# TINY-KE/DSP-SLAM-RGBD

Hardware: AMD Instinct MI355X
Metric: object-reconstructions/sec (2048 pts, 10 GN iters) (higher is better)
Workload: dtype fp16-mfma: 3xFP16 split (hi/lo fp16, fp32 accumulate) for every value that reaches an output + one-product fp16 classification of ray samples

## Files before the change

dsp-slam-rgbd_amd/csrc/dsr_api.hip:

```cpp
#include <hip/hip_runtime.h>
#include <rccl/rccl.h>
#include <dlfcn.h>

#include <algorithm>
#include <chrono>
#include <climits>
#include <cmath>
#include <cstdio>
#include <cstring>
#include <functional>
#include <map>
#include <mutex>
#include <string>
#include <thread>
#include <vector>

#include "../../include/dsr.h"
#include "dsr_kernels.hpp"
#include "dsr_mc.hpp"

#ifndef DSR_DEFAULT_FWD_VARIANT
#define DSR_DEFAULT_FWD_VARIANT 12
#endif

// ... 28 lines not shown

static bool test_hooks() {
  const char* e = getenv("DSR_TEST_HOOKS");
  return e && atoi(e) != 0;
}
static const char* hook_env(const char* k) { return test_hooks() ? getenv(k) : nullptr; }

#ifndef DSR_DEFAULT_SPLIT_RING
#define DSR_DEFAULT_SPLIT_RING 2
#endif
static int split_ring() {
  const char* e = hook_env("DSR_SPLIT_RING");
  const int r = e ? atoi(e) : DSR_DEFAULT_SPLIT_RING;
  return (r >= 2 && r <= 4) ? r : 0;
}
using FwdKernel = void (*)(DevDecoder, const Tile*, const int*, const ObjDesc*, const float4*, const float*,
                           const float*, float*, unsigned*, ErtArgs, MaskArgs);
template <int MSK>
static FwdKernel fwd16_kernel() {
  switch (split_ring()) {
    case 2: return k_mlp_fwd16<true, MSK | 1024>;
    case 3: return k_mlp_fwd16<true, MSK | 2048>;
    case 4: return k_mlp_fwd16<true, MSK | 3072>;
  }
  return k_mlp_fwd16<true, MSK>;
}
static FwdKernel fwd_kernel(int v) {
  switch (v & 15) {
    case 1: return k_mlp_fwd<1>;
    case 2: return k_mlp_fwd<2>;
    case 3: return k_mlp_fwd<3>;
    case 6: return k_mlp_fwd<6>;
    case 7: return k_mlp_fwd<7>;
    case 8: return k_mlp_fwd16<false, 0>;
    case 12: return fwd16_kernel<0>();
    default: return k_mlp_fwd<0>;
  }
}
using JacKernel = void (*)(DevDecoder, const Tile*, const int*, const ObjDesc*, const ObjState*, const float*,
                           const float4*, const float*, const float*, const float*, GNParams, float*,
                           const float4*, float*, float*, MaskArgs, float*);
static int jac_variant();
static JacKernel jac_kernel() {
  const int v = jac_variant();
  switch (v) {
    case 8: return k_mlp_jac16<false, 0>;
    case 12:
      switch (split_ring()) {
        case 2: return k_mlp_jac16<true, 2>;
        case 3: return k_mlp_jac16<true, 3>;
        case 4: return k_mlp_jac16<true, 4>;
      }
      return k_mlp_jac16<true, 0>;
  }
  return k_mlp_jac;
}
static bool is_variant(const DevDecoder& D) { return D.xyz_all || D.use_tanh || D.ln_mask; }
static FwdKernel fwd_kernel_for(const DevDecoder& D, int v) {
  return is_variant(D) ? k_mlp_fwd16<true, 1024 | 8192> : fwd_kernel(v);
}
static JacKernel jac_kernel_for(const DevDecoder& D) {
  return is_variant(D) ? k_mlp_jac16<true, 2, true> : jac_kernel();
}
using LiteKernel = void (*)(DevDecoder, const Tile*, const int*, const ObjDesc*, const float4*, const float*,
// ... 116 lines not shown
  uint64_t *rbits = nullptr, *abits = nullptr;
  MaskArgs ma{nullptr, nullptr, nullptr, nullptr};
  int* kslot = nullptr;
  bool lite = true;
  int loop_iters = 0;
  bool spare_run = false;
  ErtArgs lite_cfg{};
  bool hooks = false;
  int* diag = nullptr;
  std::vector<int> passes;
  std::vector<hipEvent_t> ev;
  bool ran = false;
  int runs = 0;
  bool timed = false;
  bool prescan = false;
  int ran_fwd = 0, ran_jac = 0, ran_lite = 0, ran_ring = 0;
#ifdef DSR_EXP_PROV
  int *prov_alive = nullptr, *prov_set = nullptr, *prov_xcc = nullptr, *prov_j = nullptr;
  unsigned* prov_t = nullptr;
  unsigned* prov_h = nullptr;
  unsigned* prov_ri = nullptr;
  float* prov_nrm = nullptr;
  float* prov_nrm2 = nullptr;
  float* prov_y = nullptr;
  int prov_R = 0, prov_C = 0;
#endif
  hipGraphExec_t graph = nullptr;
  long graph_key = -1;
  int captures = 0, replays = 0;
  bool capacity = false;
  bool cap_graph = false;
// ... 1060 lines not shown
  return 0;
}

static int batch_enqueue(dsr_batch* b, bool timing = true);
static int batch_finish(dsr_batch* b);

static int jac_variant() {
  const char* e = hook_env("DSR_JAC_VARIANT");
  return e ? atoi(e) : 12;
}

static bool graph_enabled() {
  const char* ge = getenv("DSR_GRAPH");
  return ge && atoi(ge) != 0;
}
static long graph_key() { return ((long)fwd_variant() * 100000 + jac_variant()) * 10 + split_ring(); }

static int batch_capture(dsr_batch* b) {
  dsr_ctx* ctx = b->ctx;
  if (b->graph) {
    hipGraphExecDestroy(b->graph);
    b->graph = nullptr;
  }
  hipGraph_t g = nullptr;
  DSR_CHECK(ctx, hipStreamBeginCapture(ctx->stream, hipStreamCaptureModeThreadLocal));
  const int rc = batch_enqueue(b, false);
  const hipError_t ec = hipStreamEndCapture(ctx->stream, &g);
  if (rc) {
    if (g) hipGraphDestroy(g);
    return rc;
  }
// ... 113 lines not shown
  const GNParams P = b->P;
  const int grid = ctx->n_cu;
  const int cb = (n + 63) / 64;
  const int fv = fwd_variant();
  const FwdKernel fwdk = fwd_kernel_for(D, fv);
  const JacKernel jack = jac_kernel_for(D);
  const LiteKernel litek = lite_kernel();
  {
    const int fl = fv & 15;
    const bool known = fl == 1 || fl == 2 || fl == 3 || fl == 6 || fl == 7 || fl == 8 || fl == 12;
    const int jv = jac_variant();
    b->ran_fwd = is_variant(D) ? 12 : (known ? fv : (fv & ~15));
    b->ran_jac = is_variant(D) ? 12 : ((jv == 8 || jv == 12) ? jv : 0);
    b->ran_lite = b->lite ? lite_variant_dispatched() : 0;
    b->ran_ring = is_variant(D) ? 2 : split_ring();
  }
  const int np = (int)b->passes.size() - 1;
  const size_t epi = ev_per_iter(b);
  const int G = (int)b->groups.size();
  DSR_CHECK(ctx, hipEventRecord(b->fork_ev, s0));
  for (int g = 1; g < G; ++g) DSR_CHECK(ctx, hipStreamWaitEvent(ctx->gstream[g], b->fork_ev, 0));
  for (int it = it0; it < it1; ++it) {
    for (int g = 0; g < G; ++g) {
      const dsr_batch::Group& gr = b->groups[g];
      hipStream_t s = ctx->gstream[g];
      const int ng = gr.n, o0 = gr.o0;
      const ObjDesc* desc = b->desc + o0;
      ObjState* st = b->st + o0;
      float* zbuf = b->zbuf + (size_t)o0 * CODE;
      float* b0 = b->bias0f + (size_t)o0 * HID;
// ... 161 lines not shown
  st->lite_eligible = b->dec->info.lite_eligible;
  st->audit = (b->lite && b->lite_cfg.audit) ? 1 : 0;
  st->audit_shell = b->lite_cfg.shell;
  st->audit_log2 = b->lite_cfg.audit_log2;
  st->lite_margin0 = b->P.lite_margin0;
  st->lite_floor = b->P.lite_floor;
  st->lite_safety = b->P.lite_safety;
  st->graph_captures = b->captures;
  st->graph_replays = b->replays;
  st->n_groups = (int)b->groups.size();
  st->graph_mode = b->cap_graph ? 2 : (graph_enabled() ? 1 : 0);
  st->fwd_variant = b->ran_fwd;
  st->jac_variant = b->ran_jac;
  st->lite_variant = b->ran_lite;
  st->split_ring = b->ran_ring;
  st->prescan = b->prescan ? 1 : 0;
  {
    int nb = 0;
    DSR_CHECK(b->ctx, hipMemcpy(&nb, b->diag + STD_BROKEN, sizeof(int), hipMemcpyDeviceToHost));
    st->lite_broken_blocks = nb;
  }
  st->keep_masks = (b->lite && b->ma.msk && b->ran_fwd == 12) ? 1 : 0;
  st->surface_in_exact = (st->keep_masks && b->ma.pts && b->ran_jac == 12) ? 1 : 0;
  if (b->lite) {
    st->lite_min_margin = 1e30;
    for (const ObjState& o : hs) {
      st->lite_max_err = std::max(st->lite_max_err, (double)o.lite_err);
      if (o.iters_done > 0) st->lite_min_margin = std::min(st->lite_min_margin, (double)o.lite_margin);
      st->lite_audit_violations += o.lite_viol_total;
      st->lite_redo_objects += o.lite_redo ? 1 : 0;
// ... 834 lines not shown
```

dsp-slam-rgbd_amd/csrc/dsr_kernels.hpp:

```cpp
#pragma once
#include "dsr_dev.hpp"
#include "dsr_mlp.hpp"
#include "dsr_mlp16.hpp"
#include "dsr_mlp_lite.hpp"
#include "../../include/dsr.h"

extern "C" __device__ __attribute__((const)) unsigned long long __ockl_wfred_max_u64(unsigned long long);

namespace dsr {

template <int N>
__device__ __forceinline__ void lu_small(float (&a)[N][N], int (&piv)[N]) {
#pragma unroll
  for (int k = 0; k < N; ++k) {
    int p = k;
    float best = fabsf(a[k][k]);
#pragma unroll
    for (int r = k + 1; r < N; ++r)
      if (fabsf(a[r][k]) > best) { best = fabsf(a[r][k]); p = r; }
    piv[k] = p;
#pragma unroll
    for (int r = k + 1; r < N; ++r) {
      const bool sw = (p == r);
#pragma unroll
// ... 1314 lines not shown
  }
}

struct Jac16Shared {
  _Float16 Hh[TILE * PH];
  _Float16 Hl[TILE * PH];
  float xyz[TILE * 4];
  float red[NWAVE * TILE];
  float red2[NWAVE * TILE];
  float y[TILE];
  float r[TILE];
  float gin[TILE * GIN_PITCH];
  float wmax[NWAVE];
};

#if defined(DSR_EXP_NOLS)
constexpr int BWD_LS = 0;
#elif defined(DSR_EXP_BLS1)
constexpr int BWD_LS = 1;
#else
constexpr int BWD_LS = 2;
#endif

#ifdef DSR_EXP_STAMP
#define JSTAMP(cat)                                                         \
  {                                                                         \
    __builtin_amdgcn_sched_barrier(0);                                      \
    const unsigned long long t_ = __builtin_amdgcn_s_memtime();            \
    jstamp[cat] += t_ - jstamp_last;                                        \
    jstamp_last = t_;                                                       \
    __builtin_amdgcn_sched_barrier(0);                                      \
  }
#else
#define JSTAMP(cat)
#endif
template <bool PRIO, int NB, bool VAR = false>
__global__ __launch_bounds__(512) void k_mlp_jac16(DevDecoder D, const Tile* __restrict__ tiles,
                                                   const int* __restrict__ n_tiles,
                                                   const ObjDesc* __restrict__ desc,
                                                   const ObjState* __restrict__ st,
                                                   const float* __restrict__ pts_all,
                                                   const float4* __restrict__ kpts,
                                                   const float* __restrict__ kres,
                                                   const float* __restrict__ bias0f,
                                                   const float* __restrict__ bias4f, GNParams P,
                                                   float* __restrict__ slots,
                                                   const float4* __restrict__ raw_pts,
                                                   float* __restrict__ raw_out,
                                                   float* __restrict__ res_out, MaskArgs MA,
                                                   float* __restrict__ lnws) {
  __shared__ Jac16Shared sm;
  const int w = __builtin_amdgcn_readfirstlane(threadIdx.x >> 6);
  float* const lnw = lnws ? lnws + (size_t)blockIdx.x * LN_WS_WG : nullptr;
  const int nt = *n_tiles;
#ifdef DSR_EXP_STAMP
  unsigned long long jstamp[8] = {0, 0, 0, 0, 0, 0, 0, 0};
  unsigned long long jstamp_last = __builtin_amdgcn_s_memtime();
  int jtiles = 0;
#endif
  for (int ti = blockIdx.x; ti < nt; ti += gridDim.x) {
    const Tile tl = tiles[ti];
    const ObjDesc d = desc[tl.obj];
#ifdef DSR_EXP_STAMP
    ++jtiles;
#endif
    float zpre = 0.f;
    {
      const int tid = opaque(threadIdx.x);
      if (tid < TILE) {
        float x = 0.f, y = 0.f, z = 0.f, aux = 0.f, rr = 0.f;
        zpre = bias0f[tl.obj * HID];
        if (tid < tl.count) {
          if (tl.term == 0) {
            const float* p = pts_all + (size_t)(d.pts_off + tl.start + tid) * 3;
            const float3 xo = xform(st[tl.obj].T, p[0], p[1], p[2]);
            x = xo.x; y = xo.y; z = xo.z;
          } else if (tl.term == 1) {
            const float4 v = kpts[d.cand_off + tl.start + tid];
            x = v.x; y = v.y; z = v.z; aux = v.w;
            rr = kres[d.cand_off + tl.start + tid];
          } else {
            const float4 v = raw_pts[tl.start + tid];
// ... 2 lines not shown
        }
        *reinterpret_cast<float4*>(sm.xyz + tid * 4) = make_float4(x, y, z, aux);
        sm.r[tid] = rr;
      }
    }
    __syncthreads();
    uint64_t mk[8];
    float v[4][4][4];
    floatx4 acc[4][4];
    int sa;
    Scales2 fs;
    bool fast = false;
    if (MA.kslot != nullptr && tl.term == 1) {
      const int tid = opaque(threadIdx.x);
      int bad = 0;
      if (tid < tl.count) bad = MA.kslot[d.cand_off + tl.start + tid] < 0;
      fast = !__syncthreads_or(bad);
    } else if (MA.pts != nullptr && tl.term == 0) {
      fast = true;
    }
    auto mslot = [&](int p) {
      return tl.term == 1 ? d.cand_off + MA.kslot[d.cand_off + tl.start + p] : MA.surf_base + d.pts_off + tl.start + p;
    };
    if (fast) {
      const int lane = opaque(threadIdx.x & 63), g = lane >> 4, c = lane & 15;
#pragma unroll
      for (int l = 0; l < 8; ++l) mk[l] = 0;
#pragma unroll
      for (int cb = 0; cb < 4; ++cb) {
        const int p = 16 * cb + c;
        if (p < tl.count) {
          const uint4 m4 = *reinterpret_cast<const uint4*>(MA.msk + (size_t)mslot(p) * 256 + (w * 4 + g) * 8);
          const unsigned dw[4] = {m4.x, m4.y, m4.z, m4.w};
#pragma unroll
          for (int l = 0; l < 8; ++l) {
            const unsigned u = (dw[l >> 1] >> (16 * (l & 1))) & 0xFFFFu;
#pragma unroll
            for (int q = 0; q < 4; ++q) mk[l] |= (uint64_t)((u >> (4 * q)) & 0xFu) << (16 * q + 4 * cb);
          }
        }
      }
      const int tid = opaque(threadIdx.x);
      if (tid < TILE) sm.y[tid] = (tid < tl.count) ? MA.yv[mslot(tid)] : 0.f;
      __syncthreads();
      JSTAMP(0)
    } else {
      JSTAMP(0)
      {
        const int lane = opaque(threadIdx.x & 63), g = lane >> 4, c = lane & 15;
        const float* bias0 = bias0f + tl.obj * HID;
        float m = 0.f;
        mk[0] = 0;
#pragma unroll
        for (int q = 0; q < 4; ++q) {
          const int n0 = 64 * w + 16 * q + 4 * g;
          const float4 bb = *reinterpret_cast<const float4*>(bias0 + n0);
          float wx[12];
#pragma unroll
// ... 110 lines not shown
          float y = tanhf(s + D.b8);
          if (VAR && D.use_tanh) y = tanhf(y);
          sm.y[tid] = y;
        }
      }
      __syncthreads();
    }
    float xg[4][3] = {{0.f, 0.f, 0.f}, {0.f, 0.f, 0.f}, {0.f, 0.f, 0.f}, {0.f, 0.f, 0.f}};
    const bool xlane = VAR && D.xyz_all && w == 7 && ((threadIdx.x & 63) >> 4) == 3;
    {
      const int lane = opaque(threadIdx.x & 63), g = lane >> 4, c = lane & 15;
      float m = 0.f;
#pragma unroll
      for (int q = 0; q < 4; ++q) {
        const int n0 = 64 * w + 16 * q + 4 * g;
        const float4 w8 = *reinterpret_cast<const float4*>(D.W8 + n0);
#pragma unroll
        for (int cb = 0; cb < 4; ++cb) {
          const int p = 16 * cb + c;
          const float yy = sm.y[p];
          float dt = 1.f - yy * yy;
          if (VAR && D.use_tanh) {
            const float t = atanhf(yy);
            dt = dt * (1.f - t * t);
          }
#pragma unroll
          for (int r = 0; r < 4; ++r) {
            const float gv = ((mk[7] >> ((q * 4 + cb) * 4 + r)) & 1ull) ? dt * fetch4(w8, r) : 0.f;
            v[q][cb][r] = gv;
            m = fmaxf(m, fabsf(gv));
            if (q == 3 && r >= 1 && xlane) xg[cb][r - 1] = dt * fetch4(w8, r);
// ... 3 lines not shown
      if (VAR && ((D.ln_mask >> 7) & 1))
        m = ln_bwd(v, D.ln_g[7], D.ln_dim[7], sm.red, sm.red2, w, lane, lnw + (size_t)7 * LN_WS_LAYER);
      JSTAMP(7)
      sa = block_scale(m, sm.wmax, w, lane);
      JSTAMP(3)
      write_split(v, sa, sm.Hh, sm.Hl, w, lane);
      JSTAMP(4)
    }
    __syncthreads();
    JSTAMP(5)
#pragma unroll 1
    for (int l = 7; l >= 1; --l) {
      const int lane = opaque(threadIdx.x & 63), g = lane >> 4, c = lane & 15;
      gemm16_sel<PRIO, NB, BWD_LS>(D.Wbh_raw[l], w, D.Kb[l] / 32, sm.Hh, sm.Hl, acc, lane);
      JSTAMP(1)
      const float usc = ldexpf(1.f, -(D.swb[l] + sa));
      float m = 0.f;
      const uint64_t mask = mk[l - 1];
      [&]<int... K>(std::integer_sequence<int, K...>) {
        ([&] {
          constexpr int q = K >> 4, cb = (K >> 2) & 3, r = K & 3;
          const float gv = keep_if<K>(accr(acc[q][cb], r) * (usc * rc_sign(q, cb)), mask);
          v[q][cb][r] = gv;
          m = fmaxf(m, fabsf(gv));
        }(), ...);
      }(std::make_integer_sequence<int, 64>{});
      if (xlane && l != 4) {
#pragma unroll
        for (int cb = 0; cb < 4; ++cb)
#pragma unroll
// ... 637 lines not shown
```

dsp-slam-rgbd_amd/csrc/dsr_mlp.hpp:

```cpp
#pragma once
#include "dsr_dev.hpp"

namespace dsr {

constexpr int H_FLOATS = TILE * PITCH;

template <int NQ>
__device__ __forceinline__ void mfma_step(const float4 (&a)[NQ], const float4 (&b)[4],
                                          floatx4 (&acc)[NQ][4]) {
#pragma unroll
  for (int j = 0; j < 4; ++j)
#pragma unroll
    for (int q = 0; q < NQ; ++q)
#pragma unroll
      for (int cb = 0; cb < 4; ++cb)
        acc[q][cb] = __builtin_amdgcn_mfma_f32_16x16x4f32(fetch4(a[q], j), fetch4(b[cb], j),
                                                          acc[q][cb], 0, 0, 0);
}

template <int NQ>
__device__ __forceinline__ void gemm_tile(const float4* __restrict__ A, int T,
                                          const float* __restrict__ Hs,
                                          floatx4 (&acc)[NQ][4], int lane) {
#pragma unroll
// ... 126 lines not shown
        v[r] = relu_t(accr(acc[q][cb], r) + fetch4(bb, r));
        if (relu_pass(v[r])) mask |= 1ull << ((q * 4 + cb) * 4 + r);
      }
      if (is_l3 && n0 == l3 - 1) {
        v[1] = xyz[p * 4 + 0];
        v[2] = xyz[p * 4 + 1];
        v[3] = xyz[p * 4 + 2];
      }
      *reinterpret_cast<float4*>(Hs + p * PITCH + n0) = make_float4(v[0], v[1], v[2], v[3]);
    }
  }
}

__device__ __forceinline__ void epi_l7(floatx4 (&acc)[4][4], const DevDecoder& D, float* red,
                                       int w, int lane, uint64_t& mask, const float* xyz = nullptr,
                                       bool with_bias = true) {
  const int g = lane >> 4, c = lane & 15;
  mask = 0;
  float part[4] = {0.f, 0.f, 0.f, 0.f};
  const bool xr = D.xyz_all && xyz != nullptr && w == 7;
#pragma unroll
  for (int q = 0; q < 4; ++q) {
    const int n0 = 64 * w + 16 * q + 4 * g;
    const float4 bb = with_bias ? *reinterpret_cast<const float4*>(D.bias[7] + n0) : make_float4(0.f, 0.f, 0.f, 0.f);
    const float4 w8 = *reinterpret_cast<const float4*>(D.W8 + n0);
#pragma unroll
    for (int cb = 0; cb < 4; ++cb) {
      float4 p = make_float4(0.f, 0.f, 0.f, 0.f);
      const bool on = xr && q == 3 && g == 3;
      if (q == 3 && xr) p = *reinterpret_cast<const float4*>(xyz + (16 * cb + c) * 4);
#pragma unroll
      for (int r = 0; r < 4; ++r) {
        float v = relu_t(accr(acc[q][cb], r) + fetch4(bb, r));
        if (relu_pass(v)) mask |= 1ull << ((q * 4 + cb) * 4 + r);
        if (r >= 1) v = on ? (r == 1 ? p.x : (r == 2 ? p.y : p.z)) : v;
        part[cb] = __builtin_fmaf(fetch4(w8, r), v, part[cb]);
      }
    }
  }
#pragma unroll
// ... 56 lines not shown
```

dsp-slam-rgbd_amd/csrc/dsr_mlp16.hpp:

```cpp
#pragma once
#include <utility>
#include "dsr_dev.hpp"
#include "dsr_mlp.hpp"

namespace dsr {

typedef _Float16 half8 __attribute__((ext_vector_type(8)));
typedef _Float16 half4 __attribute__((ext_vector_type(4)));

constexpr int PH = 528;

#if defined(DSR_LITE_EXPERIMENTS) || defined(DSR_EXP_NOSIGN)
constexpr bool SPLIT_ROW_SIGNS = false;
#else
constexpr bool SPLIT_ROW_SIGNS = true;
#endif
__device__ __forceinline__ constexpr float row_sign(int q) { return (SPLIT_ROW_SIGNS && (q & 1)) ? -1.f : 1.f; }
#ifdef DSR_EXP_COLSIGN
__device__ __forceinline__ constexpr float col_sign(int cb) { return (SPLIT_ROW_SIGNS && (cb & 1)) ? -1.f : 1.f; }
#else
__device__ __forceinline__ constexpr float col_sign(int) { return 1.f; }
#endif
__device__ __forceinline__ constexpr float rc_sign(int q, int cb) { return row_sign(q) * col_sign(cb); }

struct Fwd16Shared {
  _Float16 Hh[TILE * PH];
  _Float16 Hl[TILE * PH];
  float xyz[TILE * 4];
  float red[NWAVE * TILE];
  float red2[NWAVE * TILE];
  float wmax[NWAVE];
};

__device__ __forceinline__ int h_boff(int lane) {
  const int c = lane & 15;
  return c * PH + 8 * ((lane >> 4) ^ ((c >> 2) & 1));
}

template <bool PRIO, int NQ, int EX = 0, bool LS = false>
__device__ __forceinline__ void mfma3_step(const half8 (&ah)[NQ], const half8 (&al)[NQ], const half8 (&bh)[4],
                                           const half8 (&bl)[4], floatx4 (&acc)[NQ][4]) {
  if (PRIO) __builtin_amdgcn_s_setprio(1);
  if constexpr (LS && (EX & 1) == 0) {
#pragma unroll
    for (int cb = 0; cb < 4; ++cb) {
      floatx4 lo[NQ];
#pragma unroll
// ... 618 lines not shown
  stamp(4);
  mk = bits;
  return sc;
}

template <bool PRIO, int X>
__global__ __launch_bounds__(512) void k_mlp_fwd16(DevDecoder D, const Tile* __restrict__ tiles,
                                                   const int* __restrict__ n_tiles,
                                                   const ObjDesc* __restrict__ desc,
                                                   const float4* __restrict__ cand,
                                                   const float* __restrict__ bias0f,
                                                   const float* __restrict__ bias4f,
                                                   float* __restrict__ dense, unsigned* __restrict__,
                                                   ErtArgs E, MaskArgs MA) {
  __shared__ Fwd16Shared sm;
  const int w = __builtin_amdgcn_readfirstlane(threadIdx.x >> 6);
  const int nt = *n_tiles;
  constexpr bool MSK = (X & 512) != 0;
  constexpr bool VAR = (X & 8192) != 0;
  constexpr int NB = ((X >> 10) & 3) == 0 ? 0 : 1 + ((X >> 10) & 3);
#ifdef DSR_EXP_STAMP
  unsigned long long fst[12] = {0, 0, 0, 0, 0, 0, 0, 0, 0, 0, 0, 0};
  unsigned long long fst_last = __builtin_amdgcn_s_memtime();
  int ftiles = 0;
  auto stamp = [&](int cat) {
    __builtin_amdgcn_sched_barrier(0);
    const unsigned long long t = __builtin_amdgcn_s_memtime();
    fst[cat] += t - fst_last;
    fst_last = t;
    __builtin_amdgcn_sched_barrier(0);
  };
#else
  NoStamp stamp;
#endif
  for (int ti = blockIdx.x; ti < nt; ti += gridDim.x) {
#ifdef DSR_EXP_STAMP
    ++ftiles;
#endif
    const Tile tl = tiles[ti];
    const ObjDesc d = desc[tl.obj];
    const bool surf = MSK && tl.term == 3;
    const int mbase = surf ? MA.surf_base + d.pts_off + tl.start : d.cand_off + tl.start;
    float zpre = 0.f, ylpre = 0.f;
    {
      const int tid = opaque(threadIdx.x);
      if (tid < TILE) {
        float4 v = make_float4(0.f, 0.f, 0.f, 0.f);
        zpre = bias0f[tl.obj * HID];
        if (tid < tl.count) {
          if (surf) {
            const float* p = MA.pts + (size_t)(d.pts_off + tl.start + tid) * 3;
            const float3 xo = xform(E.st[tl.obj].T, p[0], p[1], p[2]);
            v = make_float4(xo.x, xo.y, xo.z, 0.f);
          } else {
            v = cand[d.cand_off + tl.start + tid];
            if (E.st) ylpre = dense[d.cand_off + (__float_as_int(v.w) & ~AUDIT_BIT)];
          }
        }
        *reinterpret_cast<float4*>(sm.xyz + tid * 4) = v;
      }
    }
    __syncthreads();
    stamp(0);
    Scales2 sa;
    MaskQueue mq;
    {
      const int lane = opaque(threadIdx.x & 63), g = lane >> 4, c = lane & 15;
      const float* bias0 = bias0f + tl.obj * HID;
      float v[4][4][4];
      float m = 0.f;
#pragma unroll
      for (int q = 0; q < 4; ++q) {
        const int n0 = 64 * w + 16 * q + 4 * g;
        const float4 bb = *reinterpret_cast<const float4*>(bias0 + n0);
        float wx[12];
#pragma unroll
        for (int i = 0; i < 12; ++i) wx[i] = D.W0x[n0 * 3 + i];
#pragma unroll
        for (int cb = 0; cb < 4; ++cb) {
          const float4 p = *reinterpret_cast<const float4*>(sm.xyz + (16 * cb + c) * 4);
#pragma unroll
          for (int r = 0; r < 4; ++r)
            v[q][cb][r] = fetch4(bb, r) + ((wx[3 * r] * p.x + wx[3 * r + 1] * p.y) + wx[3 * r + 2] * p.z);
// ... 13 lines not shown
      if constexpr (MSK) b0 = relu_bits(v);
      if (VAR && D.xyz_all && w == 7) xyz_rows(v, sm.xyz, lane, m, 3);
      sa = block_scale2(m, sm.wmax, w, lane);
      write_split(v, sa.of(w), sm.Hh, sm.Hl, w, lane);
      if constexpr (MSK) mask_push(mq, b0);
    }
    __syncthreads();
    floatx4 acc[4][4];
#pragma unroll 1
    for (int l = 1; l <= 6; ++l) {
      const int lane = opaque(threadIdx.x & 63);
      stamp(7);
      if (SURF_LS != FWD_LS && surf) gemm16_sel<PRIO, NB, SURF_LS>(D.Wh_raw[l], w, D.Kf[l] / 32, sm.Hh, sm.Hl, acc, lane, sa.resc());
      else gemm16_sel<PRIO, NB, FWD_LS>(D.Wh_raw[l], w, D.Kf[l] / 32, sm.Hh, sm.Hl, acc, lane, sa.resc());
      stamp(1);
      uint64_t mk;
      sa = epi16(acc, D.sw[l] + sa.b, (l == 4) ? bias4f + tl.obj * HID : D.bias[l], sm, w, lane, mk,
                 VAR ? xyz_row(D, l) : (l == 3 ? D.l3 : -1), stamp, VAR ? &D : nullptr, l);
      if constexpr (MSK) mask_push(mq, mk);
      stamp(7);
      __syncthreads();
      stamp(5);
    }
    {
      const int lane = opaque(threadIdx.x & 63);
      stamp(7);
      if (SURF_LS != FWD_LS && surf) gemm16_sel<PRIO, NB, SURF_LS>(D.Wh_raw[7], w, D.Kf[7] / 32, sm.Hh, sm.Hl, acc, lane, sa.resc());
      else gemm16_sel<PRIO, NB, FWD_LS>(D.Wh_raw[7], w, D.Kf[7] / 32, sm.Hh, sm.Hl, acc, lane, sa.resc());
      stamp(1);
      const int un = D.sw[7] + sa.b;
#pragma unroll
      for (int q = 0; q < 4; ++q)
#pragma unroll
        for (int cb = 0; cb < 4; ++cb)
#pragma unroll
          for (int r = 0; r < 4; ++r) acc[q][cb][r] = ldexpf(acc[q][cb][r], -un) * rc_sign(q, cb);
      uint64_t mask;
      const bool ln7 = VAR && ((D.ln_mask >> 7) & 1);
      if (ln7) ln_l7(acc, D, sm.red, sm.red2, w, lane, nullptr);
      epi_l7(acc, D, sm.red, w, lane, mask, VAR ? sm.xyz : nullptr, !ln7);
      if constexpr (MSK) {
        mask_push(mq, mask);
        mask_store(mq, MA.msk, mbase, tl.count, w, lane);
      }
      stamp(8);
    }
    __syncthreads();
    stamp(9);
    {
      const int tid = opaque(threadIdx.x);
      float emax = 0.f;
      if (tid < tl.count) {
        float s = sm.red[tid];
        for (int k = 1; k < NWAVE; ++k) s += sm.red[k * TILE + tid];
        float y = tanhf(s + D.b8);
        if (VAR && D.use_tanh) y = tanhf(y);
        stamp(10);
        const float4 p = *reinterpret_cast<const float4*>(sm.xyz + tid * 4);
        const float zprobe = zpre;
        if (p.x != p.x || p.y != p.y || p.z != p.z || zprobe != zprobe) y = __builtin_nanf("");
        if (surf) {
          MA.yv[mbase + tid] = y;
        } else {
// ... 9 lines not shown
              if (cl != ce) atomicAdd(&E.st[tl.obj].lite_viol, 1);
            }
          }
          dense[d.cand_off + idx] = y;
          if constexpr (MSK) MA.yv[d.cand_off + tl.start + tid] = y;
          if (E.dead && y <= E.nth) dead_put(E.dead + d.ray_off + idx / E.M, 1);
        }
      }
      stamp(11);
      if (w == 0 && E.st && !surf) {
        emax = wave_max(emax, opaque(threadIdx.x & 63));
        if ((threadIdx.x & 63) == 0 && emax > 0.f)
          atomicMax(reinterpret_cast<int*>(&E.st[tl.obj].lite_err), __float_as_int(emax));
      }
    }
    __syncthreads();
    stamp(6);
  }
#ifdef DSR_EXP_STAMP
  if (blockIdx.x < 4 && (threadIdx.x == 0 || threadIdx.x == 256))
    printf("fwd16_stamp %d %d %d %llu %llu %llu %llu %llu %llu %llu %llu %llu %llu %llu %llu\n", (int)blockIdx.x, w,
           ftiles, fst[0], fst[1], fst[2], fst[3], fst[4], fst[5], fst[6], fst[7], fst[8], fst[9], fst[10], fst[11]);
#endif
}

}
```

dsp-slam-rgbd_amd/reconstruct/_libdsr.py:

```python
from __future__ import annotations

import ctypes as C
import os
import threading

import numpy as np

_HERE = os.path.dirname(os.path.abspath(__file__))
_PKG = os.path.dirname(_HERE)
DEFAULT_LIB = os.path.join(_PKG, "csrc", "libdsr.so")

MAX_LAYERS = 16
CODE_LEN = 64
FAIL_REASONS = {0: "ok", 1: "sdf loss is NaN", 2: "fewer than 10 ray samples in the unit ball",
                3: "render loss is NaN (no render points)"}


class DsrError(RuntimeError):
    pass


FP = C.POINTER(C.c_float)
IP = C.POINTER(C.c_int)

# ... 24 lines not shown
                ("loss", C.c_float), ("is_good", C.c_int), ("fail_reason", C.c_int),
                ("iters_done", C.c_int), ("n_valid_last", C.c_int), ("k_last", C.c_int)]


class PoseIn(C.Structure):
    _fields_ = [("t_co_se3", C.c_float * 16), ("scale", C.c_float), ("pts", FP), ("n_pts", C.c_int),
                ("code", FP)]


class Trace(C.Structure):
    _fields_ = [("H", FP), ("b", FP), ("dx", FP), ("loss", FP), ("sdf_loss", FP),
                ("render_loss", FP), ("n_valid", IP), ("k", IP), ("t_obj_cam", FP), ("z", FP),
                ("n_decoded", IP), ("n_refined", IP)]


ABI_VERSION = 11
BATCH_GRAPH = 1
GATHER_HOST, GATHER_RCCL = 0, 1


class Stats(C.Structure):
    _fields_ = [("fwd_ms", C.c_double), ("jac_ms", C.c_double), ("total_ms", C.c_double),
                ("fwd_points", C.c_int64), ("jac_points", C.c_int64),
                ("fwd_launches", C.c_int), ("jac_launches", C.c_int), ("inball_points", C.c_int64),
                ("lite", C.c_int), ("refine_launches", C.c_int), ("refine_ms", C.c_double),
                ("refine_points", C.c_int64), ("lite_max_err", C.c_double),
                ("lite_min_margin", C.c_double), ("jac_surface_points", C.c_int64),
                ("jac_render_points", C.c_int64), ("keep_masks", C.c_int),
                ("lite_audit_violations", C.c_int), ("lite_redo_objects", C.c_int),
                ("surface_in_exact", C.c_int), ("audit_points", C.c_int64),
                ("lite_broken_blocks", C.c_int), ("test_hooks", C.c_int),
                ("lite_eligible", C.c_int), ("audit", C.c_int), ("audit_shell", C.c_float),
                ("audit_log2", C.c_int), ("lite_margin0", C.c_float), ("lite_floor", C.c_float),
                ("lite_safety", C.c_float), ("graph_captures", C.c_int), ("graph_replays", C.c_int),
                ("n_groups", C.c_int), ("graph_mode", C.c_int), ("fwd_variant", C.c_int),
                ("jac_variant", C.c_int), ("lite_variant", C.c_int), ("split_ring", C.c_int),
                ("prescan", C.c_int)]


class DecoderInfo(C.Structure):
    _fields_ = [("code_len", C.c_int), ("lite_eligible", C.c_int), ("lite_probe_ratio", C.c_double),
                ("lite_probe_max_err", C.c_double), ("lite_probe_max_err_all", C.c_double),
                ("probe_points", C.c_int), ("probe_codes", C.c_int), ("probe_ms", C.c_double)]

LITE_DIAG_FIELDS = ("broken_blocks", "recorded", "block", "wave", "counter", "target", "observed", "tile_iter",
                    "hw_id", "xcc_id", "polls", "real_ticks")
LITE_DIAG_COUNTERS = ("ovf0", "ovf1", "cH0", "cH1", "cRlo", "cRhi", "cP", "cT0", "cT1", "cE", "broken")
LITE_DIAG_INTS = len(LITE_DIAG_FIELDS)


SIGNATURES = {
    "dsr_abi_version": (C.c_int, []),
# ... 136 lines not shown
```

include/dsr.h:

```cpp
#ifndef DSR_H
#define DSR_H

#include <stddef.h>
#include <stdint.h>

#ifdef __cplusplus
extern "C" {
#endif

#define DSR_ABI_VERSION 11
#define DSR_MAX_LAYERS 16
#define DSR_CODE_LEN 64

typedef struct dsr_ctx dsr_ctx;
typedef struct dsr_decoder dsr_decoder;
typedef struct dsr_batch dsr_batch;

typedef struct {
  int code_len;
  int n_layers;
  int out_dim[DSR_MAX_LAYERS];
  int in_dim[DSR_MAX_LAYERS];
  int latent_in;
  int use_tanh;
  int xyz_in_all;
// ... 83 lines not shown
  int audit;
  float audit_shell;
  int audit_log2;
  float lite_margin0;
  float lite_floor;
  float lite_safety;
  int graph_captures;
  int graph_replays;
  int n_groups;
  int graph_mode;
  int fwd_variant;
  int jac_variant;
  int lite_variant;
  int split_ring;
  int prescan;
} dsr_stats;

int dsr_abi_version(void);
int dsr_ctx_create(int device, dsr_ctx** out);
int dsr_ctx_destroy(dsr_ctx* ctx);
const char* dsr_last_error(const dsr_ctx* ctx);
int dsr_device_count(int* n);

int dsr_decoder_load(dsr_ctx* ctx, const dsr_decoder_desc* desc, const float* weights,
                     size_t n_floats, dsr_decoder** out);
int dsr_decoder_free(dsr_ctx* ctx, dsr_decoder* dec);

typedef struct {
  int code_len;
  int lite_eligible;
// ... 71 lines not shown
```

Measured before the change: 382.4.

## Prefetch next tile descriptors and inputs into LDS during MLP layers

Adds a tile-prefetch path to the fp16 forward and Jacobian kernels. While the current tile's middle GEMM layers run, wave 0 issues global-to-LDS loads (global_load_lds) for the next tile's descriptor, object descriptor, point inputs, biases and mask slots. Constant biases and W8 are also staged into shared memory once per block. This is meant to hide the dependent global-load latency at each tile start, and the trailing barrier is dropped. The cost is extra LDS, extra waits inside the layer loop, and a mask store moved after the barrier. The path is on by default for split ring 2.

```diff
diff --git a/dsp-slam-rgbd_amd/csrc/dsr_api.hip b/dsp-slam-rgbd_amd/csrc/dsr_api.hip
--- a/dsp-slam-rgbd_amd/csrc/dsr_api.hip
+++ b/dsp-slam-rgbd_amd/csrc/dsr_api.hip
@@ -66,12 +66,16 @@
   const int r = e ? atoi(e) : DSR_DEFAULT_SPLIT_RING;
   return (r >= 2 && r <= 4) ? r : 0;
 }
+static bool tile_prefetch() {
+  const char* e = hook_env("DSR_TILE_PREFETCH");
+  return !(e && atoi(e) == 0);
+}
 using FwdKernel = void (*)(DevDecoder, const Tile*, const int*, const ObjDesc*, const float4*, const float*,
                            const float*, float*, unsigned*, ErtArgs, MaskArgs);
 template <int MSK>
 static FwdKernel fwd16_kernel() {
   switch (split_ring()) {
-    case 2: return k_mlp_fwd16<true, MSK | 1024>;
+    case 2: return tile_prefetch() ? k_mlp_fwd16<true, MSK | 1024 | 16384> : k_mlp_fwd16<true, MSK | 1024>;
     case 3: return k_mlp_fwd16<true, MSK | 2048>;
     case 4: return k_mlp_fwd16<true, MSK | 3072>;
   }
@@ -99,7 +103,7 @@
     case 8: return k_mlp_jac16<false, 0>;
     case 12:
       switch (split_ring()) {
-        case 2: return k_mlp_jac16<true, 2>;
+        case 2: return tile_prefetch() ? k_mlp_jac16<true, 2, false, true> : k_mlp_jac16<true, 2>;
         case 3: return k_mlp_jac16<true, 3>;
         case 4: return k_mlp_jac16<true, 4>;
       }
@@ -246,7 +250,7 @@
   int runs = 0;
   bool timed = false;
   bool prescan = false;
-  int ran_fwd = 0, ran_jac = 0, ran_lite = 0, ran_ring = 0;
+  int ran_fwd = 0, ran_jac = 0, ran_lite = 0, ran_ring = 0, ran_pf = 0;
 #ifdef DSR_EXP_PROV
   int *prov_alive = nullptr, *prov_set = nullptr, *prov_xcc = nullptr, *prov_j = nullptr;
   unsigned* prov_t = nullptr;
@@ -1337,7 +1341,9 @@
   const char* ge = getenv("DSR_GRAPH");
   return ge && atoi(ge) != 0;
 }
-static long graph_key() { return ((long)fwd_variant() * 100000 + jac_variant()) * 10 + split_ring(); }
+static long graph_key() {
+  return (((long)fwd_variant() * 100000 + jac_variant()) * 10 + split_ring()) * 2 + (tile_prefetch() ? 1 : 0);
+}
 
 static int batch_capture(dsr_batch* b) {
   dsr_ctx* ctx = b->ctx;
@@ -1481,6 +1487,7 @@
     b->ran_jac = is_variant(D) ? 12 : ((jv == 8 || jv == 12) ? jv : 0);
     b->ran_lite = b->lite ? lite_variant_dispatched() : 0;
     b->ran_ring = is_variant(D) ? 2 : split_ring();
+    b->ran_pf = (tile_prefetch() && !is_variant(D) && split_ring() == 2 && (fl == 12 || jv == 12)) ? 1 : 0;
   }
   const int np = (int)b->passes.size() - 1;
   const size_t epi = ev_per_iter(b);
@@ -1672,6 +1679,7 @@
   st->jac_variant = b->ran_jac;
   st->lite_variant = b->ran_lite;
   st->split_ring = b->ran_ring;
+  st->tile_prefetch = b->ran_pf;
   st->prescan = b->prescan ? 1 : 0;
   {
     int nb = 0;
diff --git a/dsp-slam-rgbd_amd/csrc/dsr_kernels.hpp b/dsp-slam-rgbd_amd/csrc/dsr_kernels.hpp
--- a/dsp-slam-rgbd_amd/csrc/dsr_kernels.hpp
+++ b/dsp-slam-rgbd_amd/csrc/dsr_kernels.hpp
@@ -1352,6 +1352,46 @@
   float wmax[NWAVE];
 };
 
+struct alignas(16) Jac16Next {
+  float xyz[TILE * 4];
+  float r[TILE];
+  int ks[TILE];
+  float y[TILE];
+  float z[TILE];
+  float T[16];
+  Tile tn;
+  ObjDesc dn;
+  float w8[HID];
+};
+__device__ __forceinline__ void jac16_next_inputs(Jac16Next& n, const ObjState* st, const float* pts_all,
+                                                  const float4* kpts, const float* kres, const float* bias0f,
+                                                  const float4* raw_pts, const MaskArgs& MA, int lane) {
+  const Tile t = n.tn;
+  const ObjDesc d = n.dn;
+  glds4(bias0f + t.obj * HID, n.z);
+  if (t.term == 0 && lane < 16) glds4(st[t.obj].T + lane, n.T);
+  if (lane >= t.count) return;
+  if (t.term == 0) {
+    const float* p = pts_all + (size_t)(d.pts_off + t.start + lane) * 3;
+    glds4(p, n.xyz);
+    glds4(p + 1, n.xyz + TILE);
+    glds4(p + 2, n.xyz + 2 * TILE);
+    if (MA.pts != nullptr) glds4(MA.yv + MA.surf_base + d.pts_off + t.start + lane, n.y);
+  } else if (t.term == 1) {
+    glds16(kpts + d.cand_off + t.start + lane, n.xyz);
+    glds4(kres + d.cand_off + t.start + lane, n.r);
+    if (MA.kslot != nullptr) glds4(MA.kslot + d.cand_off + t.start + lane, n.ks);
+  } else {
+    glds16(raw_pts + t.start + lane, n.xyz);
+  }
+}
+__device__ __forceinline__ void jac16_next_kept(Jac16Next& n, const MaskArgs& MA, int lane) {
+  const Tile t = n.tn;
+  if (MA.kslot == nullptr || t.term != 1 || lane >= t.count) return;
+  const int ks = n.ks[lane];
+  if (ks >= 0) glds4(MA.yv + n.dn.cand_off + ks, n.y);
+}
+
 #if defined(DSR_EXP_NOLS)
 constexpr int BWD_LS = 0;
 #elif defined(DSR_EXP_BLS1)
@@ -1372,7 +1412,7 @@
 #else
 #define JSTAMP(cat)
 #endif
-template <bool PRIO, int NB, bool VAR = false>
+template <bool PRIO, int NB, bool VAR = false, bool PF = false>
 __global__ __launch_bounds__(512) void k_mlp_jac16(DevDecoder D, const Tile* __restrict__ tiles,
                                                    const int* __restrict__ n_tiles,
                                                    const ObjDesc* __restrict__ desc,
@@ -1388,22 +1428,61 @@
                                                    float* __restrict__ res_out, MaskArgs MA,
                                                    float* __restrict__ lnws) {
   __shared__ Jac16Shared sm;
+  __shared__ Jac16Next nx;
   const int w = __builtin_amdgcn_readfirstlane(threadIdx.x >> 6);
   float* const lnw = lnws ? lnws + (size_t)blockIdx.x * LN_WS_WG : nullptr;
   const int nt = *n_tiles;
+  if constexpr (PF) {
+    if ((int)blockIdx.x >= nt) return;
+    nx.w8[opaque(threadIdx.x)] = D.W8[opaque(threadIdx.x)];
+    if (w == 0) {
+      const int lane = opaque(threadIdx.x & 63);
+      next_tile(tiles, blockIdx.x, nx.tn, lane);
+      glds_wait();
+      next_desc(desc, nx.tn, nx.dn, lane);
+      glds_wait();
+      jac16_next_inputs(nx, st, pts_all, kpts, kres, bias0f, raw_pts, MA, lane);
+      glds_wait();
+      jac16_next_kept(nx, MA, lane);
+      glds_wait();
+    }
+    __syncthreads();
+  }
 #ifdef DSR_EXP_STAMP
   unsigned long long jstamp[8] = {0, 0, 0, 0, 0, 0, 0, 0};
   unsigned long long jstamp_last = __builtin_amdgcn_s_memtime();
   int jtiles = 0;
 #endif
   for (int ti = blockIdx.x; ti < nt; ti += gridDim.x) {
-    const Tile tl = tiles[ti];
-    const ObjDesc d = desc[tl.obj];
+    const Tile tl = PF ? tile_uniform(nx.tn) : tiles[ti];
+    const ObjDesc d = PF ? desc_uniform(nx.dn) : desc[tl.obj];
+    const bool more = PF && ti + (int)gridDim.x < nt;
 #ifdef DSR_EXP_STAMP
     ++jtiles;
 #endif
     float zpre = 0.f;
-    {
+    if constexpr (PF) {
+      const int tid = opaque(threadIdx.x);
+      if (tid < TILE) {
+        float x = 0.f, y = 0.f, z = 0.f, aux = 0.f, rr = 0.f;
+        zpre = nx.z[tid];
+        if (tid < tl.count) {
+          if (tl.term == 0) {
+            const float3 xo = xform(nx.T, nx.xyz[tid], nx.xyz[TILE + tid], nx.xyz[2 * TILE + tid]);
+            x = xo.x; y = xo.y; z = xo.z;
+          } else {
+            const float4 v = *reinterpret_cast<const float4*>(nx.xyz + tid * 4);
+            x = v.x; y = v.y; z = v.z;
+            if (tl.term == 1) {
+              aux = v.w;
+              rr = nx.r[tid];
+            }
+          }
+        }
+        *reinterpret_cast<float4*>(sm.xyz + tid * 4) = make_float4(x, y, z, aux);
+        sm.r[tid] = rr;
+      }
+    } else {
       const int tid = opaque(threadIdx.x);
       if (tid < TILE) {
         float x = 0.f, y = 0.f, z = 0.f, aux = 0.f, rr = 0.f;
@@ -1436,13 +1515,14 @@
     if (MA.kslot != nullptr && tl.term == 1) {
       const int tid = opaque(threadIdx.x);
       int bad = 0;
-      if (tid < tl.count) bad = MA.kslot[d.cand_off + tl.start + tid] < 0;
+      if (tid < tl.count) bad = (PF ? nx.ks[tid] : MA.kslot[d.cand_off + tl.start + tid]) < 0;
       fast = !__syncthreads_or(bad);
     } else if (MA.pts != nullptr && tl.term == 0) {
       fast = true;
     }
     auto mslot = [&](int p) {
-      return tl.term == 1 ? d.cand_off + MA.kslot[d.cand_off + tl.start + p] : MA.surf_base + d.pts_off + tl.start + p;
+      return tl.term == 1 ? d.cand_off + (PF ? nx.ks[p] : MA.kslot[d.cand_off + tl.start + p])
+                          : MA.surf_base + d.pts_off + tl.start + p;
     };
     if (fast) {
       const int lane = opaque(threadIdx.x & 63), g = lane >> 4, c = lane & 15;
@@ -1463,7 +1543,7 @@
         }
       }
       const int tid = opaque(threadIdx.x);
-      if (tid < TILE) sm.y[tid] = (tid < tl.count) ? MA.yv[mslot(tid)] : 0.f;
+      if (tid < TILE) sm.y[tid] = (tid < tl.count) ? (PF ? nx.y[tid] : MA.yv[mslot(tid)]) : 0.f;
       __syncthreads();
       JSTAMP(0)
     } else {
@@ -1604,7 +1684,7 @@
 #pragma unroll
       for (int q = 0; q < 4; ++q) {
         const int n0 = 64 * w + 16 * q + 4 * g;
-        const float4 w8 = *reinterpret_cast<const float4*>(D.W8 + n0);
+        const float4 w8 = *reinterpret_cast<const float4*>((PF ? nx.w8 : D.W8) + n0);
 #pragma unroll
         for (int cb = 0; cb < 4; ++cb) {
           const int p = 16 * cb + c;
@@ -1638,6 +1718,15 @@
       const int lane = opaque(threadIdx.x & 63), g = lane >> 4, c = lane & 15;
       gemm16_sel<PRIO, NB, BWD_LS>(D.Wbh_raw[l], w, D.Kb[l] / 32, sm.Hh, sm.Hl, acc, lane);
       JSTAMP(1)
+      if constexpr (PF) {
+        if (more && w == 0 && l >= 4) {
+          if (l == 7) next_tile(tiles, ti + gridDim.x, nx.tn, lane);
+          else if (l == 6) next_desc(desc, nx.tn, nx.dn, lane);
+          else if (l == 5) jac16_next_inputs(nx, st, pts_all, kpts, kres, bias0f, raw_pts, MA, lane);
+          else jac16_next_kept(nx, MA, lane);
+          glds_wait();
+        }
+      }
       const float usc = ldexpf(1.f, -(D.swb[l] + sa));
       float m = 0.f;
       const uint64_t mask = mk[l - 1];
diff --git a/dsp-slam-rgbd_amd/csrc/dsr_mlp.hpp b/dsp-slam-rgbd_amd/csrc/dsr_mlp.hpp
--- a/dsp-slam-rgbd_amd/csrc/dsr_mlp.hpp
+++ b/dsp-slam-rgbd_amd/csrc/dsr_mlp.hpp
@@ -164,16 +164,19 @@
 
 __device__ __forceinline__ void epi_l7(floatx4 (&acc)[4][4], const DevDecoder& D, float* red,
                                        int w, int lane, uint64_t& mask, const float* xyz = nullptr,
-                                       bool with_bias = true) {
+                                       bool with_bias = true,
+                                       const float* b7 = nullptr, const float* w8p = nullptr) {
   const int g = lane >> 4, c = lane & 15;
   mask = 0;
   float part[4] = {0.f, 0.f, 0.f, 0.f};
   const bool xr = D.xyz_all && xyz != nullptr && w == 7;
-#pragma unroll
-  for (int q = 0; q < 4; ++q) {
-    const int n0 = 64 * w + 16 * q + 4 * g;
-    const float4 bb = with_bias ? *reinterpret_cast<const float4*>(D.bias[7] + n0) : make_float4(0.f, 0.f, 0.f, 0.f);
-    const float4 w8 = *reinterpret_cast<const float4*>(D.W8 + n0);
+  if (b7 == nullptr) b7 = D.bias[7];
+  if (w8p == nullptr) w8p = D.W8;
+#pragma unroll
+  for (int q = 0; q < 4; ++q) {
+    const int n0 = 64 * w + 16 * q + 4 * g;
+    const float4 bb = with_bias ? *reinterpret_cast<const float4*>(b7 + n0) : make_float4(0.f, 0.f, 0.f, 0.f);
+    const float4 w8 = *reinterpret_cast<const float4*>(w8p + n0);
 #pragma unroll
     for (int cb = 0; cb < 4; ++cb) {
       float4 p = make_float4(0.f, 0.f, 0.f, 0.f);
diff --git a/dsp-slam-rgbd_amd/csrc/dsr_mlp16.hpp b/dsp-slam-rgbd_amd/csrc/dsr_mlp16.hpp
--- a/dsp-slam-rgbd_amd/csrc/dsr_mlp16.hpp
+++ b/dsp-slam-rgbd_amd/csrc/dsr_mlp16.hpp
@@ -31,6 +31,77 @@
   float red2[NWAVE * TILE];
   float wmax[NWAVE];
 };
+
+__device__ __forceinline__ void glds4(const void* g, void* lds_base) {
+  __builtin_amdgcn_global_load_lds((const __attribute__((address_space(1))) void*)g,
+                                   (__attribute__((address_space(3))) void*)lds_base, 4, 0, 0);
+}
+__device__ __forceinline__ void glds16(const void* g, void* lds_base) {
+  __builtin_amdgcn_global_load_lds((const __attribute__((address_space(1))) void*)g,
+                                   (__attribute__((address_space(3))) void*)lds_base, 16, 0, 0);
+}
+__device__ __forceinline__ void glds_wait() { asm volatile("s_waitcnt vmcnt(0)" ::: "memory"); }
+__device__ __forceinline__ int sgpr(int v) { return __builtin_amdgcn_readfirstlane(v); }
+__device__ __forceinline__ Tile tile_uniform(const Tile& t) {
+  Tile r;
+  r.obj = sgpr(t.obj); r.term = sgpr(t.term); r.start = sgpr(t.start); r.count = sgpr(t.count);
+  return r;
+}
+__device__ __forceinline__ ObjDesc desc_uniform(const ObjDesc& s) {
+  ObjDesc r;
+  r.pts_off = sgpr(s.pts_off); r.n_pts = sgpr(s.n_pts); r.ray_off = sgpr(s.ray_off); r.n_rays = sgpr(s.n_rays);
+  r.n_fg = sgpr(s.n_fg); r.cand_off = sgpr(s.cand_off); r.slot_sdf = sgpr(s.slot_sdf); r.pad = 0;
+  return r;
+}
+static_assert(sizeof(Tile) == 16 && sizeof(ObjDesc) == 32, "descriptor images are 16-byte LDS-DMA pieces");
+
+struct alignas(16) Fwd16Next {
+  float xyz[TILE * 4];
+  float b0[HID];
+  float b4[HID];
+  float yl[TILE];
+  float T[16];
+  Tile tn;
+  ObjDesc dn;
+};
+
+struct alignas(16) Fwd16Const {
+  float bias[6][HID];
+  float w8[HID];
+};
+__device__ __forceinline__ constexpr int const_row(int l) { return l < 4 ? l - 1 : l - 2; }
+
+__device__ __forceinline__ void next_tile(const Tile* tiles, int ti, Tile& tn, int lane) {
+  if (lane == 0) glds16(tiles + ti, &tn);
+}
+__device__ __forceinline__ void next_desc(const ObjDesc* desc, const Tile& tn, ObjDesc& dn, int lane) {
+  const int obj = tn.obj;
+  if (lane < 2) glds16(reinterpret_cast<const char*>(desc + obj) + 16 * lane, &dn);
+}
+template <bool MSK>
+__device__ __forceinline__ void fwd16_next_inputs(Fwd16Next& n, const float4* cand, const ErtArgs& E,
+                                                  const MaskArgs& MA, int lane) {
+  const Tile t = n.tn;
+  const ObjDesc d = n.dn;
+  if (MSK && t.term == 3) {
+    if (lane < t.count) {
+      const float* p = MA.pts + (size_t)(d.pts_off + t.start + lane) * 3;
+      glds4(p, n.xyz);
+      glds4(p + 1, n.xyz + TILE);
+      glds4(p + 2, n.xyz + 2 * TILE);
+    }
+    if (lane < 16) glds4(E.st[t.obj].T + lane, n.T);
+  } else if (lane < t.count) {
+    glds16(cand + d.cand_off + t.start + lane, n.xyz);
+  }
+}
+template <bool MSK>
+__device__ __forceinline__ void fwd16_next_lite(Fwd16Next& n, const float* dense, const ErtArgs& E, int lane) {
+  const Tile t = n.tn;
+  if (E.st == nullptr || (MSK && t.term == 3) || lane >= t.count) return;
+  const int idx = __float_as_int(n.xyz[lane * 4 + 3]) & ~AUDIT_BIT;
+  glds4(dense + n.dn.cand_off + idx, n.yl);
+}
 
 __device__ __forceinline__ int h_boff(int lane) {
   const int c = lane & 15;
@@ -679,10 +750,40 @@
                                                    float* __restrict__ dense, unsigned* __restrict__,
                                                    ErtArgs E, MaskArgs MA) {
   __shared__ Fwd16Shared sm;
+  __shared__ Fwd16Next nx;
+  __shared__ Fwd16Const cs;
   const int w = __builtin_amdgcn_readfirstlane(threadIdx.x >> 6);
   const int nt = *n_tiles;
   constexpr bool MSK = (X & 512) != 0;
   constexpr bool VAR = (X & 8192) != 0;
+  constexpr bool PF = (X & 16384) != 0;
+  auto next_bias = [&] {
+    const int row = nx.tn.obj * HID + 64 * w + opaque(threadIdx.x & 63);
+    glds4(bias0f + row, nx.b0 + 64 * w);
+    glds4(bias4f + row, nx.b4 + 64 * w);
+  };
+  if constexpr (PF) {
+    if ((int)blockIdx.x >= nt) return;
+    for (int e = opaque(threadIdx.x); e < 7 * HID; e += 512) {
+      const int k = e / HID, n = e - k * HID;
+      if (k < 6) cs.bias[k][n] = D.bias[k < 3 ? k + 1 : k + 2][n];
+      else cs.w8[n] = D.W8[n];
+    }
+    if (w == 0) {
+      const int lane = opaque(threadIdx.x & 63);
+      next_tile(tiles, blockIdx.x, nx.tn, lane);
+      glds_wait();
+      next_desc(desc, nx.tn, nx.dn, lane);
+      glds_wait();
+      fwd16_next_inputs<MSK>(nx, cand, E, MA, lane);
+      glds_wait();
+      fwd16_next_lite<MSK>(nx, dense, E, lane);
+      glds_wait();
+    }
+    __syncthreads();
+    next_bias();
+    glds_wait();
+  }
   constexpr int NB = ((X >> 10) & 3) == 0 ? 0 : 1 + ((X >> 10) & 3);
 #ifdef DSR_EXP_STAMP
   unsigned long long fst[12] = {0, 0, 0, 0, 0, 0, 0, 0, 0, 0, 0, 0};
@@ -702,12 +803,29 @@
 #ifdef DSR_EXP_STAMP
     ++ftiles;
 #endif
-    const Tile tl = tiles[ti];
-    const ObjDesc d = desc[tl.obj];
+    const Tile tl = PF ? tile_uniform(nx.tn) : tiles[ti];
+    const ObjDesc d = PF ? desc_uniform(nx.dn) : desc[tl.obj];
+    const bool more = PF && ti + (int)gridDim.x < nt;
     const bool surf = MSK && tl.term == 3;
     const int mbase = surf ? MA.surf_base + d.pts_off + tl.start : d.cand_off + tl.start;
     float zpre = 0.f, ylpre = 0.f;
-    {
+    if constexpr (PF) {
+      const int tid = opaque(threadIdx.x);
+      if (tid < TILE) {
+        float4 v = make_float4(0.f, 0.f, 0.f, 0.f);
+        zpre = nx.b0[0];
+        if (tid < tl.count) {
+          if (surf) {
+            const float3 xo = xform(nx.T, nx.xyz[tid], nx.xyz[TILE + tid], nx.xyz[2 * TILE + tid]);
+            v = make_float4(xo.x, xo.y, xo.z, 0.f);
+          } else {
+            v = *reinterpret_cast<const float4*>(nx.xyz + tid * 4);
+            if (E.st) ylpre = nx.yl[tid];
+          }
+        }
+        *reinterpret_cast<float4*>(sm.xyz + tid * 4) = v;
+      }
+    } else {
       const int tid = opaque(threadIdx.x);
       if (tid < TILE) {
         float4 v = make_float4(0.f, 0.f, 0.f, 0.f);
@@ -731,7 +849,7 @@
     MaskQueue mq;
     {
       const int lane = opaque(threadIdx.x & 63), g = lane >> 4, c = lane & 15;
-      const float* bias0 = bias0f + tl.obj * HID;
+      const float* bias0 = PF ? nx.b0 : bias0f + tl.obj * HID;
       float v[4][4][4];
       float m = 0.f;
 #pragma unroll
@@ -775,11 +893,25 @@
       if (SURF_LS != FWD_LS && surf) gemm16_sel<PRIO, NB, SURF_LS>(D.Wh_raw[l], w, D.Kf[l] / 32, sm.Hh, sm.Hl, acc, lane, sa.resc());
       else gemm16_sel<PRIO, NB, FWD_LS>(D.Wh_raw[l], w, D.Kf[l] / 32, sm.Hh, sm.Hl, acc, lane, sa.resc());
       stamp(1);
+      if constexpr (PF) {
+        if (more && w == 0) {
+          if (l == 1) next_tile(tiles, ti + gridDim.x, nx.tn, lane);
+          else if (l == 2) next_desc(desc, nx.tn, nx.dn, lane);
+          else if (l == 3) fwd16_next_inputs<MSK>(nx, cand, E, MA, lane);
+          else if (l == 4) fwd16_next_lite<MSK>(nx, dense, E, lane);
+          if (l <= 4) glds_wait();
+        }
+        if (more && l == 5) next_bias();
+      }
       uint64_t mk;
-      sa = epi16(acc, D.sw[l] + sa.b, (l == 4) ? bias4f + tl.obj * HID : D.bias[l], sm, w, lane, mk,
+      const float* bias = PF ? (l == 4 ? nx.b4 : cs.bias[const_row(l)]) : (l == 4 ? bias4f + tl.obj * HID : D.bias[l]);
+      sa = epi16(acc, D.sw[l] + sa.b, bias, sm, w, lane, mk,
                  VAR ? xyz_row(D, l) : (l == 3 ? D.l3 : -1), stamp, VAR ? &D : nullptr, l);
       if constexpr (MSK) mask_push(mq, mk);
       stamp(7);
+      if constexpr (PF) {
+        if (more && l == 5) glds_wait();
+      }
       __syncthreads();
       stamp(5);
     }
@@ -799,15 +931,18 @@
       uint64_t mask;
       const bool ln7 = VAR && ((D.ln_mask >> 7) & 1);
       if (ln7) ln_l7(acc, D, sm.red, sm.red2, w, lane, nullptr);
-      epi_l7(acc, D, sm.red, w, lane, mask, VAR ? sm.xyz : nullptr, !ln7);
+      epi_l7(acc, D, sm.red, w, lane, mask, VAR ? sm.xyz : nullptr, !ln7, PF ? cs.bias[5] : nullptr,
+             PF ? cs.w8 : nullptr);
       if constexpr (MSK) {
         mask_push(mq, mask);
-        mask_store(mq, MA.msk, mbase, tl.count, w, lane);
+        if constexpr (!PF) mask_store(mq, MA.msk, mbase, tl.count, w, lane);
       }
       stamp(8);
     }
     __syncthreads();
     stamp(9);
+    if constexpr (PF && MSK)
+      mask_store(mq, MA.msk, mbase, tl.count, w, opaque(threadIdx.x & 63));
     {
       const int tid = opaque(threadIdx.x);
       float emax = 0.f;
@@ -847,7 +982,7 @@
           atomicMax(reinterpret_cast<int*>(&E.st[tl.obj].lite_err), __float_as_int(emax));
       }
     }
-    __syncthreads();
+    if constexpr (!PF) __syncthreads();
     stamp(6);
   }
 #ifdef DSR_EXP_STAMP
diff --git a/dsp-slam-rgbd_amd/reconstruct/_libdsr.py b/dsp-slam-rgbd_amd/reconstruct/_libdsr.py
--- a/dsp-slam-rgbd_amd/reconstruct/_libdsr.py
+++ b/dsp-slam-rgbd_amd/reconstruct/_libdsr.py
@@ -62,7 +62,7 @@
                 ("n_decoded", IP), ("n_refined", IP)]
 
 
-ABI_VERSION = 11
+ABI_VERSION = 12
 BATCH_GRAPH = 1
 GATHER_HOST, GATHER_RCCL = 0, 1
 
@@ -83,7 +83,7 @@
                 ("lite_safety", C.c_float), ("graph_captures", C.c_int), ("graph_replays", C.c_int),
                 ("n_groups", C.c_int), ("graph_mode", C.c_int), ("fwd_variant", C.c_int),
                 ("jac_variant", C.c_int), ("lite_variant", C.c_int), ("split_ring", C.c_int),
-                ("prescan", C.c_int)]
+                ("prescan", C.c_int), ("tile_prefetch", C.c_int)]
 
 
 class DecoderInfo(C.Structure):
diff --git a/include/dsr.h b/include/dsr.h
--- a/include/dsr.h
+++ b/include/dsr.h
@@ -8,7 +8,7 @@
 extern "C" {
 #endif
 
-#define DSR_ABI_VERSION 11
+#define DSR_ABI_VERSION 12
 #define DSR_MAX_LAYERS 16
 #define DSR_CODE_LEN 64
 
@@ -122,6 +122,7 @@
   int lite_variant;
   int split_ring;
   int prescan;
+  int tile_prefetch;
 } dsr_stats;
 
 int dsr_abi_version(void);
```

Result: no change. 384.5 (median of 6 runs) (+0.5%).
